# votnhan/VN_celeb_face_recognition

Measured on AMD Instinct MI355X. Metric: embeddings/sec @ bs=256 (InceptionResnetV1, 160x160), higher is better.
Workload: dtype bf16

## Files before the change

### vn_celeb_face_recognition_amd/csrc/conv_device.h

```cpp
#pragma once
#include <atomic>

#include "kernels.h"
#include "split_f16.h"

namespace vnf {

typedef __bf16 bf16x8_t __attribute__((ext_vector_type(8)));
typedef _Float16 f16x8_t __attribute__((ext_vector_type(8)));
typedef float f32x4_t __attribute__((ext_vector_type(4)));

struct KArgs {
  const char* x;
  const char* w;
  const float* bias;
  const int4* ktab;
  const char* res;
  const float* slope;
  const char* zero;
  int ldx, H, W, Ho, Wo, sh, sw, ph, pw;
  int K, Kpad, nkt;
  int wrs, wts;
  int ncls, cout_pad;
  int M, Cout, tiles_n, nblk;
// ... 324 lines not shown
  } else {
    for (int pass = 0; pass < EPASS; ++pass) {
      if ((wm * WTM) / RPP == pass) {
        const int rbase = wm * WTM - pass * RPP;
#pragma unroll
        for (int i = 0; i < TM; ++i)
#pragma unroll
          for (int j = 0; j < TN; ++j)
            *reinterpret_cast<f32x4_t*>(sC + (rbase + i * 16 + frow) * CST + wn * WTN + j * 16 + fgrp * 4) = acc[i][j];
      }
      __syncthreads();
#pragma unroll
      for (int it = 0; it < NIT; ++it) {
        const int idx = tid + it * NT;
        const int r = idx / CPR, cc = idx - r * CPR;
        const int m = m0 + pass * RPP + r, c = n0 + cc * 8;
        if (idx < RPP * CPR && m < a.M && c < a.Cout) {
          int sg = 0;
#pragma unroll
          for (int s = 1; s < 4; ++s)
            if (s < a.nseg && c >= a.seg_c0[s]) sg = s;
          float v[8];
          const f32x4_t v0 = *reinterpret_cast<const f32x4_t*>(sC + r * CST + cc * 8);
          const f32x4_t v1 = *reinterpret_cast<const f32x4_t*>(sC + r * CST + cc * 8 + 4);
          int cls = 0;
          if (a.ncls == 9) {
            const int rr = m % HoWo, ho = rr / a.Wo, wo = rr - ho * a.Wo;
            cls = (ho == 0 ? 0 : (ho == a.Ho - 1 ? 2 : 1)) * 3 + (wo == 0 ? 0 : (wo == a.Wo - 1 ? 2 : 1));
          }
          const float* bp = a.bias + (size_t)cls * a.cout_pad + c;
          const f32x4_t b0 = *reinterpret_cast<const f32x4_t*>(bp), b1 = *reinterpret_cast<const f32x4_t*>(bp + 4);
#pragma unroll
          for (int e = 0; e < 4; ++e) { v[e] = v0[e] + b0[e]; v[4 + e] = v1[e] + b1[e]; }
          if (a.res) {
            float rv[8];
            load8<T>(a.res + ((size_t)m * a.ldres + c) * ES, rv);
#pragma unroll
            for (int e = 0; e < 8; ++e) v[e] += rv[e];
          }
          if (a.act == ACT_RELU) {
#pragma unroll
            for (int e = 0; e < 8; ++e) v[e] = fmaxf(v[e], 0.f);
          } else if (a.act == ACT_PRELU) {
#pragma unroll
            for (int e = 0; e < 8; ++e) v[e] = v[e] > 0.f ? v[e] : v[e] * a.slope[c + e];
          }
          char* const dptr = a.seg_ptr[sg];
          if (a.out_f32)
            store8<float>(dptr + ((size_t)m * a.seg_ld[sg] + (c - a.seg_c0[sg])) * 4, v);
          else
            store8<T>(dptr + ((size_t)m * a.seg_ld[sg] + (c - a.seg_c0[sg])) * ES, v);
        }
      }
      __syncthreads();
    }
  }
}

__device__ __forceinline__ void glds16(const void* gsrc, unsigned lds_base) {
  unsigned keep;
  asm volatile(
      "s_mov_b32 %0, m0\n\ts_mov_b32 m0, %2\n\ts_nop 0\n\tglobal_load_lds_dwordx4 %1, off\n\ts_mov_b32 m0, %0"
      : "=&s"(keep)
      : "v"(gsrc), "s"(lds_base)
      : "memory");
}

template <int N>
__device__ __forceinline__ void wait_dma_and_barrier() {
  asm volatile("s_waitcnt vmcnt(%0) lgkmcnt(0)\n\ts_barrier" ::"n"(N) : "memory");
}

constexpr int patch_epi_bytes(int bm, int bn, int wm) {
  return bm * (bn + 4) * 4 <= 64 * 1024 ? bm * (bn + 4) * 4 : (bm / wm) * (bn + 4) * 4;
}
int patch_num_cfgs();
bool patch_cfg_ok(const ConvArgs& a, int pcfg);
hipError_t launch_patch(const ConvArgs& a, const KArgs& k, int pcfg, hipStream_t s);

int ws_num_cfgs();
bool ws_cfg_ok(const ConvArgs& a, int wcfg);
hipError_t launch_ws(const ConvArgs& a, const KArgs& k, int wcfg, hipStream_t s);

}
```

### vn_celeb_face_recognition_amd/csrc/conv_igemm.hip

```cpp
#include <mutex>
#include <type_traits>

#include "block35.h"
#include "conv_device.h"

namespace vnf {

template <int AP, int RS>
__device__ __forceinline__ void row_setup(const KArgs& a, int m0, int lrow, int (&abase)[AP], int (&ahi)[AP],
                                          int (&awi)[AP]) {
  const int HoWo = a.Ho * a.Wo;
#pragma unroll
  for (int p = 0; p < AP; ++p) {
    const int m = m0 + lrow + RS * p;
    if (m < a.M) {
      const int n = m / HoWo, r = m - n * HoWo;
      const int ho = r / a.Wo, wo = r - ho * a.Wo;
      ahi[p] = ho * a.sh - a.ph;
      awi[p] = wo * a.sw - a.pw;
      abase[p] = ((n * a.H + ahi[p]) * a.W + awi[p]) * a.ldx;
    } else {
      ahi[p] = -(1 << 24);
      awi[p] = 0;
      abase[p] = 0;
// ... 172 lines not shown
      rd(kt, 1, xf[1], wf[1]);
#pragma unroll
      for (int i = 0; i < TM; ++i)
#pragma unroll
        for (int j = 0; j < TN; ++j) mma_hh(acc[i][j], wh[c][j], xh[c][i]);
    };
    int kt = 0;
    for (; kt + 1 < nkt; kt += 2) {
      step(std::integral_constant<int, 0>{}, kt);
      step(std::integral_constant<int, 1>{}, kt + 1);
    }
    if (kt < nkt) {
      step(std::integral_constant<int, 0>{}, kt);
#pragma unroll
      for (int i = 0; i < TM; ++i)
#pragma unroll
        for (int j = 0; j < TN; ++j) mma_cross(acc[i][j], wh[0][j], wf[1][j], xh[0][i], xf[1][i]);
    } else {
#pragma unroll
      for (int i = 0; i < TM; ++i)
#pragma unroll
        for (int j = 0; j < TN; ++j) mma_cross(acc[i][j], wh[1][j], wf[1][j], xh[1][i], xf[1][i]);
    }
  } else {
    bool pend = false;
    for (int kt = 0; kt < nkt; ++kt) {
      sync_tile(kt);
      read_frags(kt, 0);
      if (pend) mma(1);
      pend = BKE / 2 < a.K - kt * BKE;
      if (pend) read_frags(kt, 1);
      mma(0);
    }
    if (pend) mma(1);
  }
  __syncthreads();
  conv_epilogue<T, BM, BN, WM, WN, S * STAGE>(a, acc, smem, m0, n0);
}

static const char* zero_page() {
  static char* z[16] = {nullptr};
  static std::once_flag once[16];
  int dev = 0;
  if (hipGetDevice(&dev) != hipSuccess || dev < 0 || dev >= 16) return nullptr;
  std::call_once(once[dev], [dev] {
    char* p = nullptr;
    if (hipMalloc((void**)&p, 256) != hipSuccess) return;
    (void)hipMemset(p, 0, 256);
    (void)hipDeviceSynchronize();
    z[dev] = p;
  });
  return z[dev];
}

const char* conv_zero_page() { return zero_page(); }

template <typename T, int BM, int BN, int WM, int WN, int S>
static hipError_t launch_dma(const KArgs& k, hipStream_t s) {
  allow_dynamic_lds<conv_igemm_dma_kernel<T, BM, BN, WM, WN, S>>(160 * 1024);
  KArgs kk = k;
  const int lds = S * (BM + BN) * 128;
  const int tiles_m = (k.M + BM - 1) / BM;
  kk.tiles_n = (k.Cout + BN - 1) / BN;
  kk.nblk = tiles_m * kk.tiles_n;
  hipLaunchKernelGGL((conv_igemm_dma_kernel<T, BM, BN, WM, WN, S>), dim3(kk.nblk), dim3(WM * WN * 64), lds, s, kk);
  return hipGetLastError();
}

struct TileCfg { int bm, bn, wm, wn, s; };
static const TileCfg kCfgs[] = {
    {128, 128, 2, 2, 3}, {128, 64, 2, 2, 3}, {128, 32, 4, 1, 3}, {64, 64, 2, 2, 4}, {64, 32, 2, 2, 4},
    {256, 32, 4, 1, 3},  {256, 64, 4, 1, 3}, {64, 128, 1, 4, 3}, {32, 64, 2, 2, 4}, {32, 128, 1, 4, 4},
    {128, 64, 2, 2, 4},  {64, 64, 2, 2, 3},  {128, 32, 4, 1, 4},
    {128, 128, 2, 4, 3}, {256, 128, 4, 2, 3}, {256, 64, 4, 2, 3}, {128, 64, 4, 2, 3}, {128, 256, 2, 4, 3},
    {128, 128, 2, 4, 4},
    {128, 64, 4, 2, 6},  {64, 64, 2, 2, 8},   {64, 32, 2, 2, 8},  {32, 64, 2, 2, 8},  {128, 32, 4, 1, 6},
    {64, 128, 2, 4, 5},  {128, 64, 2, 2, 6},
    {64, 256, 1, 8, 3},  {64, 256, 1, 8, 4},  {128, 256, 2, 4, 3},
    {128, 96, 4, 1, 3},  {64, 96, 2, 2, 4},   {128, 192, 2, 4, 3}, {64, 192, 2, 4, 3},  {256, 96, 4, 1, 3},
    {64, 192, 2, 4, 4},
};
constexpr int kNumCfgs = (int)(sizeof(kCfgs) / sizeof(kCfgs[0]));

int conv_num_cfgs() { return kNumCfgs + patch_num_cfgs() + ws_num_cfgs(); }

static bool dma_capable(const ConvArgs& a) { return (a.Kpad / (128 / dtype_size(a.dtype))) * 8 * 16 <= 24 * 1024; }

bool conv_cfg_ok(const ConvArgs& a, int cfg) {
  if (cfg >= kNumCfgs + patch_num_cfgs()) return dma_capable(a) && ws_cfg_ok(a, cfg - kNumCfgs - patch_num_cfgs());
  if (cfg >= kNumCfgs) return dma_capable(a) && patch_cfg_ok(a, cfg - kNumCfgs);
  if (cfg < 0) return false;
  const TileCfg& c = kCfgs[cfg];
  if (c.bn > 32 && a.Cout <= c.bn / 2) return false;
  if (((a.Cout + c.bn - 1) / c.bn) * c.bn > a.cout_pad) return false;
  if ((c.bn % 64) && a.Cout % c.bn) return false;
  const int lds = c.s * (c.bm + c.bn) * 128;
  return lds <= 160 * 1024;
}

template <typename T>
static hipError_t launch_cfg(int cfg, const KArgs& k, hipStream_t s) {
  switch (cfg) {
    case 0: return launch_dma<T, 128, 128, 2, 2, 3>(k, s);
    case 1: return launch_dma<T, 128, 64, 2, 2, 3>(k, s);
    case 2: return launch_dma<T, 128, 32, 4, 1, 3>(k, s);
    case 3: return launch_dma<T, 64, 64, 2, 2, 4>(k, s);
    case 4: return launch_dma<T, 64, 32, 2, 2, 4>(k, s);
    case 5: return launch_dma<T, 256, 32, 4, 1, 3>(k, s);
    case 6: return launch_dma<T, 256, 64, 4, 1, 3>(k, s);
    case 7: return launch_dma<T, 64, 128, 1, 4, 3>(k, s);
    case 8: return launch_dma<T, 32, 64, 2, 2, 4>(k, s);
    case 9: return launch_dma<T, 32, 128, 1, 4, 4>(k, s);
    case 10: return launch_dma<T, 128, 64, 2, 2, 4>(k, s);
    case 11: return launch_dma<T, 64, 64, 2, 2, 3>(k, s);
    case 12: return launch_dma<T, 128, 32, 4, 1, 4>(k, s);
    case 13: return launch_dma<T, 128, 128, 2, 4, 3>(k, s);
    case 14: return launch_dma<T, 256, 128, 4, 2, 3>(k, s);
    case 15: return launch_dma<T, 256, 64, 4, 2, 3>(k, s);
    case 16: return launch_dma<T, 128, 64, 4, 2, 3>(k, s);
    case 17: return launch_dma<T, 128, 256, 2, 4, 3>(k, s);
    case 18: return launch_dma<T, 128, 128, 2, 4, 4>(k, s);
    case 19: return launch_dma<T, 128, 64, 4, 2, 6>(k, s);
    case 20: return launch_dma<T, 64, 64, 2, 2, 8>(k, s);
    case 21: return launch_dma<T, 64, 32, 2, 2, 8>(k, s);
    case 22: return launch_dma<T, 32, 64, 2, 2, 8>(k, s);
    case 23: return launch_dma<T, 128, 32, 4, 1, 6>(k, s);
    case 24: return launch_dma<T, 64, 128, 2, 4, 5>(k, s);
    case 25: return launch_dma<T, 128, 64, 2, 2, 6>(k, s);
    case 26: return launch_dma<T, 64, 256, 1, 8, 3>(k, s);
    case 27: return launch_dma<T, 64, 256, 1, 8, 4>(k, s);
    case 28: return launch_dma<T, 128, 256, 2, 4, 3>(k, s);
    case 29: return launch_dma<T, 128, 96, 4, 1, 3>(k, s);
    case 30: return launch_dma<T, 64, 96, 2, 2, 4>(k, s);
    case 31: return launch_dma<T, 128, 192, 2, 4, 3>(k, s);
    case 32: return launch_dma<T, 64, 192, 2, 4, 3>(k, s);
    case 33: return launch_dma<T, 256, 96, 4, 1, 3>(k, s);
    case 34: return launch_dma<T, 64, 192, 2, 4, 4>(k, s);
  }
  return hipErrorInvalidValue;
}

template <typename T>
static hipError_t launch_typed(const ConvArgs& a, const KArgs& k, hipStream_t s) {
  if (!k.zero) return hipErrorOutOfMemory;
  if (a.cfg >= kNumCfgs + patch_num_cfgs() && conv_cfg_ok(a, a.cfg)) return launch_ws(a, k, a.cfg - kNumCfgs - patch_num_cfgs(), s);
  if (a.cfg >= kNumCfgs && conv_cfg_ok(a, a.cfg)) return launch_patch(a, k, a.cfg - kNumCfgs, s);
  if (a.cfg >= 0 && conv_cfg_ok(a, a.cfg)) return launch_cfg<T>(a.cfg, k, s);
  auto fits = [&](int) { return true; };
  int bn = 128;
  while (bn > 32 && !(fits(bn) && (a.Cout % bn == 0 || a.Cout > 2 * bn))) bn >>= 1;
  if (!fits(bn)) return hipErrorInvalidValue;
  auto blocks = [&](int bm_, int bn_) { return ((a.M + bm_ - 1) / bm_) * ((a.Cout + bn_ - 1) / bn_); };
  while (bn > 64 && blocks(128, bn) < 512) bn >>= 1;
  int bm = 128;
  if (bn <= 64 && blocks(128, bn) < 512) bm = 64;
  const int id = bm == 128 ? (bn == 128 ? 0 : bn == 64 ? 1 : 2) : (bn == 64 ? 3 : 4);
  return launch_cfg<T>(id, k, s);
}

hipError_t launch_conv(const ConvArgs& a, hipStream_t s) {
  if (a.M <= 0) return hipSuccess;
  const int es = dtype_size(a.dtype);
  const int bke = 128 / es;
  if (a.Cout % 8 || a.Kpad % bke || a.nseg < 1 || a.nseg > 4) return hipErrorInvalidValue;
  KArgs k;
  k.x = (const char*)a.x; k.w = (const char*)a.w; k.bias = a.bias; k.ktab = a.ktab;
  k.res = (const char*)a.res; k.slope = a.slope; k.zero = zero_page();
  k.ldx = a.ldx; k.H = a.H; k.W = a.W; k.Ho = a.Ho; k.Wo = a.Wo;
  k.sh = a.sh; k.sw = a.sw; k.ph = a.ph; k.pw = a.pw;
  k.K = a.K; k.Kpad = a.Kpad; k.nkt = a.Kpad / bke;
  k.wrs = a.Kpad * es; k.wts = 128;
  k.ncls = a.ncls; k.cout_pad = a.cout_pad;
  k.M = a.M; k.Cout = a.Cout; k.tiles_n = 0; k.nblk = 0;
  k.ldres = a.ldres; k.act = a.act; k.out_f32 = a.out_f32;
  k.nseg = a.nseg;
  k.KH = a.KH; k.KW = a.KW; k.Cin = a.Cin; k.pp = k.Wp = k.Hv = k.patch_bytes = k.lds_bytes = 0; k.dbg = nullptr;
  for (int i = 0; i < 4; ++i) {
    k.seg_c0[i] = i < a.nseg ? a.seg[i].c0 : 1 << 30;
    k.seg_c1[i] = i < a.nseg ? a.seg[i].c1 : 1 << 30;
    k.seg_ld[i] = i < a.nseg ? a.seg[i].ld : 0;
    k.seg_ptr[i] = i < a.nseg ? (char*)a.seg[i].ptr : nullptr;
  }
  switch (a.dtype) {
    case BF16: return launch_typed<__bf16>(a, k, s);
    case F16: return launch_typed<_Float16>(a, k, s);
    case F32: return launch_typed<float>(a, k, s);
    case F16X2: return launch_typed<sf16>(a, k, s);
    case F16P: return launch_typed<pf16>(a, k, s);
  }
  return hipErrorInvalidValue;
}

}
```

### vn_celeb_face_recognition_amd/csrc/engine.cpp

```cpp
#include "engine.h"
#include "split_f16.h"
#include "block35.h"
#include "stem_mid.h"
#include "trunk17.h"

#include <algorithm>
#include <cmath>
#include <cstdio>
#include <cstdlib>
#include <cstring>
#include <map>

namespace vnf {

static thread_local std::string g_err;
void set_error(const std::string& msg) { g_err = msg; }
int fail(int code, const std::string& msg) {
  g_err = msg;
  return code;
}
const char* last_error_cstr() { return g_err.c_str(); }

HandleBase::~HandleBase() {
  for (void* p : allocs) (void)hipFree(p);
// ... 25 lines not shown
    if (w[i].name) m[w[i].name] = &w[i];
}
const float* WeightMap::get(const std::string& name, int64_t numel) {
  auto it = m.find(name);
  if (it == m.end() || it->second->dtype != VNF_F32 || !it->second->data) {
    if (missing.empty()) missing = name;
    return nullptr;
  }
  int64_t n = 1;
  for (int i = 0; i < it->second->ndim; ++i) n *= it->second->shape[i];
  if (n != numel) {
    if (missing.empty()) missing = name + " (unexpected size)";
    return nullptr;
  }
  return (const float*)it->second->data;
}

static inline uint16_t f2bf16(float f) {
  uint32_t u;
  memcpy(&u, &f, 4);
  if ((u & 0x7fffffffu) > 0x7f800000u) return (uint16_t)((u >> 16) | 0x40);
  return (uint16_t)((u + 0x7fffu + ((u >> 16) & 1u)) >> 16);
}
void convert_to(int dtype, const float* src, void* dst, size_t n) {
  if (dtype == F32) {
    memcpy(dst, src, n * 4);
  } else if (dtype == BF16) {
    uint16_t* d = (uint16_t*)dst;
    for (size_t i = 0; i < n; ++i) d[i] = f2bf16(src[i]);
  } else if (dtype == F16X2) {
    sf16* d = (sf16*)dst;
    for (size_t i = 0; i < n; ++i) d[i] = sf16(src[i]);
  } else if (dtype == F16P) {
    _Float16* d = (_Float16*)dst;
    for (size_t t = 0; t + 32 <= n; t += 32)
      for (int i = 0; i < 32; ++i) {
        const sf16 v(src[t + i]);
        d[2 * t + i] = v.hi;
        d[2 * t + 32 + i] = v.lo;
      }
  } else {
    _Float16* d = (_Float16*)dst;
    for (size_t i = 0; i < n; ++i) d[i] = (_Float16)src[i];
  }
}

int Encoder::add_buf(int H, int W, int C) {
  Buf b;
  b.H = H; b.W = W; b.C = C;
  bufs.push_back(b);
  return (int)bufs.size() - 1;
}

ConvArgs Encoder::conv_args(const ConvLayer& L, int n0, int nn) const {
  const int es = dtype_size(dtype);
  const Buf& xb = bufs[L.x_buf];
  ConvArgs a;
  memset(&a, 0, sizeof(a));
  a.dtype = dtype;
  a.x = xb.ptr + ((size_t)n0 * xb.elems_per_image() + L.x_coff) * es;
  a.ldx = xb.C; a.H = L.H; a.W = L.W; a.Cin = L.cin; a.Ho = L.Ho; a.Wo = L.Wo;
  a.KH = L.KH; a.KW = L.KW; a.sh = L.sh; a.sw = L.sw; a.ph = L.ph; a.pw = L.pw;
  a.w = L.w; a.K = L.K; a.Kpad = L.Kpad; a.bias = L.bias; a.ncls = L.ncls; a.cout_pad = L.cout_pad;
  a.ktab = L.ktab; a.M = nn * L.Ho * L.Wo; a.Cout = L.cout; a.nseg = L.nseg;
  for (int i = 0; i < L.nseg; ++i) {
    a.seg[i].c0 = L.seg[i].c0; a.seg[i].c1 = L.seg[i].c1;
    if (L.seg[i].buf == -2) {
      a.seg[i].ptr = emb_raw + (size_t)n0 * 512;
      a.seg[i].ld = 512;
    } else {
      const Buf& ob = bufs[L.seg[i].buf];
      a.seg[i].ptr = ob.ptr + ((size_t)n0 * ob.elems_per_image() + L.seg[i].coff) * (L.out_f32 ? 4 : es);
      a.seg[i].ld = ob.C;
    }
  }
  if (L.res_buf >= 0) {
    const Buf& rb = bufs[L.res_buf];
    a.res = rb.ptr + ((size_t)n0 * rb.elems_per_image() + L.res_coff) * es;
    a.ldres = rb.C;
  }
  a.act = L.act; a.slope = L.slope; a.out_f32 = L.out_f32;
  a.cfg = L.cfg;
  a.ws_persist = env.ws_persist;
  return a;
}

int Encoder::autotune() {
  const int enabled = env.autotune, force = env.force_cfg;
  if (!enabled && force < -1) return VNF_OK;
  std::map<std::string, int> cache;
  const char* cache_path = env.tune_cache.empty() ? nullptr : env.tune_cache.c_str();
  bool cache_dirty = false;
  if (cache_path && enabled) {
    if (FILE* f = fopen(cache_path, "r")) {
      char key[256];
      int c;
      while (fscanf(f, "%255s %d", key, &c) == 2) cache[key] = c;
      fclose(f);
    }
  }
  VNF_HIP(hipDeviceSynchronize());
  struct Timers {
    hipEvent_t e0 = nullptr, e1 = nullptr;
    hipStream_t lane_s[4] = {nullptr, nullptr, nullptr, nullptr};
    hipEvent_t lane_e[4] = {nullptr, nullptr, nullptr, nullptr};
    ~Timers() {
      if (e0) (void)hipEventDestroy(e0);
      if (e1) (void)hipEventDestroy(e1);
      for (int l = 0; l < 4; ++l) {
        if (lane_e[l]) (void)hipEventDestroy(lane_e[l]);
        if (lane_s[l]) (void)hipStreamDestroy(lane_s[l]);
      }
    }
  } tm;
  VNF_HIP(hipEventCreate(&tm.e0));
  VNF_HIP(hipEventCreate(&tm.e1));
  hipEvent_t e0 = tm.e0, e1 = tm.e1;
  hipStream_t* lane_s = tm.lane_s;
  hipEvent_t* lane_e = tm.lane_e;
  const int lanes = env.tune_lanes > 0 ? (env.tune_lanes > 4 ? 4 : env.tune_lanes) : (tune_lanes < 1 ? 1 : tune_lanes);
  if (lanes > 1)
    for (int l = 0; l < lanes; ++l) {
      VNF_HIP(hipStreamCreateWithFlags(&lane_s[l], hipStreamNonBlocking));
      VNF_HIP(hipEventCreate(&lane_e[l]));
    }
  for (const Group& g : groups) {
    int part = (max_batch >= 192 && max_streams > 1) ? (max_batch + 1) / 2 : max_batch;
    if (tune_batch > 0 && tune_batch < part) part = tune_batch;
    const int nn = g.chunk < part ? g.chunk : part;
    for (int oi = g.first; oi < g.last; ++oi) {
      if (ops[oi].kind != Op::CONV) continue;
      bool in_fused = false;
      for (const FusedStack& f : fused) in_fused |= f.active && oi >= f.first && oi < (f.ext ? f.ext_last : f.last);
      if (in_fused) continue;
      ConvLayer& L = convs[ops[oi].a];
      float best = 1e30f;
      int best_cfg = -1;
      char key[256];
      snprintf(key, sizeof key, "%s/d%d/n%d/M%d/K%d/N%d/v%d/L%d", L.name.c_str(), dtype, nn, nn * L.Ho * L.Wo, L.Kpad, L.cout,
               conv_num_cfgs(), lanes);
      const auto hit = cache.find(key);
      if (hit != cache.end()) {
        ConvArgs a = conv_args(L, 0, nn);
        if (hit->second == -1 || conv_cfg_ok(a, hit->second)) { L.cfg = hit->second; continue; }
      }
      std::vector<std::pair<float, int>> timed;
      auto time_cfg = [&](const ConvArgs& a, int trials, int reps, float* out_ms) -> int {
        float ms = 1e30f;
        for (int trial = 0; trial < trials; ++trial) {
          float t = 0;
          if (lanes <= 1) {
            VNF_HIP(hipEventRecord(e0, 0));
            for (int r = 0; r < reps; ++r) (void)launch_conv(a, 0);
            VNF_HIP(hipEventRecord(e1, 0));
            VNF_HIP(hipEventSynchronize(e1));
            VNF_HIP(hipEventElapsedTime(&t, e0, e1));
          } else {
            VNF_HIP(hipDeviceSynchronize());
            VNF_HIP(hipEventRecord(e0, lane_s[0]));
            for (int r = 0; r < reps; ++r)
              for (int l = 0; l < lanes; ++l) (void)launch_conv(a, lane_s[l]);
            for (int l = 0; l < lanes; ++l) VNF_HIP(hipEventRecord(lane_e[l], lane_s[l]));
            for (int l = 0; l < lanes; ++l) {
              float tl = 0;
              VNF_HIP(hipEventSynchronize(lane_e[l]));
              VNF_HIP(hipEventElapsedTime(&tl, e0, lane_e[l]));
              if (tl > t) t = tl;
            }
          }
          t *= 4.f / reps;
          if (t < ms) ms = t;
        }
        *out_ms = ms;
        return VNF_OK;
      };
      const int logit = env.autotune_log;
      for (int cfg = -1; enabled && cfg < conv_num_cfgs(); ++cfg) {
        ConvArgs a = conv_args(L, 0, nn);
        a.cfg = cfg;
        if (cfg >= 0 && !conv_cfg_ok(a, cfg)) continue;
        if (launch_conv(a, 0) != hipSuccess) { (void)hipGetLastError(); continue; }
        float ms = 1e30f;
        const int rc = time_cfg(a, 2, 4, &ms);
        if (rc != VNF_OK) return rc;
        timed.emplace_back(ms, cfg);
        if (ms < best) { best = ms; best_cfg = cfg; }
        if (logit) fprintf(stderr, "autotune %s cfg %d: %.4f ms\n", L.name.c_str(), cfg, ms / 4);
      }
      if (env.tune_final && timed.size() > 1) {
        std::sort(timed.begin(), timed.end());
        float fbest = 1e30f;
        int fcfg = best_cfg, nfin = 0;
        for (const auto& tc : timed) {
          if (tc.first > timed[0].first * 1.08f || nfin == 4) break;
          ++nfin;
          ConvArgs a = conv_args(L, 0, nn);
          a.cfg = tc.second;
          float ms = 1e30f;
          const int rc = time_cfg(a, 3, 8, &ms);
          if (rc != VNF_OK) return rc;
          if (logit) fprintf(stderr, "autotune %s final cfg %d: %.4f ms\n", L.name.c_str(), tc.second, ms / 4);
          if (ms < fbest) { fbest = ms; fcfg = tc.second; }
        }
        if (nfin > 1) { best = fbest; best_cfg = fcfg; }
      }
      L.cfg = best_cfg;
      if (cache_path && enabled) { cache[key] = best_cfg; cache_dirty = true; }
      if (force >= -1) {
        ConvArgs a = conv_args(L, 0, nn);
        if (force == -1 || conv_cfg_ok(a, force)) L.cfg = force;
      }
    }
  }
  VNF_HIP(hipDeviceSynchronize());
  if (cache_dirty) {
    if (FILE* f = fopen(cache_path, "w")) {
      for (auto& kv : cache) fprintf(f, "%s %d\n", kv.first.c_str(), kv.second);
      fclose(f);
    }
  }
  return VNF_OK;
}

int Encoder::finalize() {
  const int es = dtype_size(dtype);
  for (auto& b : bufs) {
    const size_t bytes = b.elems_per_image() * es * (size_t)max_batch;
    b.ptr = (char*)dalloc(bytes);
    if (!b.ptr) return VNF_E_HIP;
    VNF_HIP(hipMemset(b.ptr, 0, bytes));
  }
  emb_raw = (float*)dalloc((size_t)max_batch * 512 * 4);
  if (!emb_raw) return VNF_E_HIP;
  macs_alg = macs_exec = 0;
  for (auto& c : convs) { macs_alg += c.macs_alg; macs_exec += c.macs_exec; }
  if (groups.empty()) groups.push_back({0, (int)ops.size(), 1 << 30});
  {
    const int rc = prepare_fused();
    if (rc != VNF_OK) return rc;
  }
  tune_dirty = true;
  return VNF_OK;
}

EncoderEnv EncoderEnv::read() {
  auto env_int = [](const char* name, int dflt) { const char* v = getenv(name); return v ? atoi(v) : dflt; };
  EncoderEnv e;
  e.fuse = env_int("VNF_FUSE", e.fuse);
  e.direct_stem = env_int("VNF_DIRECT_STEM", e.direct_stem);
  e.stem1a_mfma = env_int("VNF_STEM1A_MFMA", e.stem1a_mfma);
  e.stem_chunk = env_int("VNF_STEM_CHUNK", e.stem_chunk);
  e.ir100_chunk1 = env_int("VNF_IR100_CHUNK1", e.ir100_chunk1);
  e.ir100_chunk2 = env_int("VNF_IR100_CHUNK2", e.ir100_chunk2);
  e.retina_fuse = env_int("VNF_RETINA_FUSE", e.retina_fuse);
  e.ws_persist = env_int("VNF_WS_PERSIST", e.ws_persist);
  e.autotune = env_int("VNF_AUTOTUNE", e.autotune);
  e.force_cfg = env_int("VNF_FORCE_CFG", e.force_cfg);
  e.tune_lanes = env_int("VNF_TUNE_LANES", e.tune_lanes);
  e.autotune_log = env_int("VNF_AUTOTUNE_LOG", e.autotune_log);
  e.tune_final = env_int("VNF_TUNE_FINAL", 1) != 0;
  if (const char* cache = getenv("VNF_TUNE_CACHE")) e.tune_cache = cache;
  return e;
}

int Encoder::prepare_fused() {
  const int enabled = env.fuse;
  for (FusedStack& f : fused) {
    f.active = false;
    if (!enabled || (dtype != BF16 && dtype != F16 && dtype != F16P) || f.nblocks < 1 || f.nblocks > T17_MAX_BLOCKS) continue;
    if (f.kind == 2) {
      if (!(enabled & 4)) continue;
      const ConvLayer& c2a = convs[f.conv0];
      const ConvLayer& c2b = convs[f.conv0 + 1];
      if (c2a.cout != 32 || c2a.K != 288 || c2b.cout != 64 || c2b.K != 288 || c2a.ncls != 1 || c2b.ncls != 1)
        return fail(VNF_E_INVALID, "fused stem: unexpected layer shapes");
      StemMidPack pk;
      pk.w[0] = c2a.w; pk.kpad[0] = c2a.Kpad;
      pk.w[1] = c2b.w; pk.kpad[1] = c2b.Kpad;
      bool ext_ok = false;
      if ((enabled & 8) && f.ext_conv >= 0) {
        const ConvLayer& c3b = convs[f.ext_conv];
        ext_ok = c3b.cout == 80 && c3b.K == 64 && c3b.KH == 1 && c3b.ncls == 1 && c3b.nseg == 1 && c3b.res_buf < 0 && c3b.act == ACT_RELU &&
                 bufs[f.ext_out_buf].C == 80;
      }
      if (dtype == F16P && !ext_ok) continue;
      f.wstream = dalloc(dtype == F16P ? SMS_WFRAG_BYTES : SM_WFRAG_BYTES);
      f.bias = (float*)dalloc(SM_BIAS * 4);
      if (!f.wstream || !f.bias) return VNF_E_HIP;
      VNF_HIP(hipMemcpy(f.bias, c2a.bias, 32 * 4, hipMemcpyDeviceToDevice));
      VNF_HIP(hipMemcpy(f.bias + 32, c2b.bias, 64 * 4, hipMemcpyDeviceToDevice));
      VNF_HIP(dtype == F16P ? stem_mids_repack(pk, f.wstream, 0) : stem_mid_repack(pk, f.wstream, 0));
      VNF_HIP(hipDeviceSynchronize());
      f.macs_alg = c2a.macs_alg + c2b.macs_alg;
      f.active = true;
      f.ext = ext_ok;
      if (ext_ok) f.macs_alg += convs[f.ext_conv].macs_alg;
      continue;
    }
    if (f.kind == 35) {
      if (!(enabled & 2)) continue;
      std::vector<float> bias((size_t)f.nblocks * B35_BIAS, 0.f);
      static const int rows[5] = {96, 32, 32, 32, 256}, ks[5] = {256, 288, 288, 288, 96}, boff[5] = {0, 96, 128, 160, 192};
      const size_t wimg_bytes = dtype == F16P ? B35S_WIMG_BYTES : B35_WIMG_BYTES;
      f.wstream = dalloc((size_t)f.nblocks * wimg_bytes);
      f.bias = (float*)dalloc(bias.size() * 4);
      if (!f.wstream || !f.bias) return VNF_E_HIP;
      for (int b = 0; b < f.nblocks; ++b) {
        Block35Pack pk;
        pk.bias = f.bias + (size_t)b * B35_BIAS;
        for (int c = 0; c < 5; ++c) {
          const ConvLayer& L = convs[f.conv0 + 5 * b + c];
          if (L.cout != rows[c] || L.K != ks[c] || L.ncls != 1) return fail(VNF_E_INVALID, "fused Block35: unexpected layer shapes");
          pk.w[c] = L.w;
          pk.kpad[c] = L.Kpad;
          VNF_HIP(hipMemcpy(&bias[(size_t)b * B35_BIAS + boff[c]], L.bias, (size_t)rows[c] * 4, hipMemcpyDeviceToHost));
          f.macs_alg += L.macs_alg;
        }
        VNF_HIP(hipMemcpy(f.bias + (size_t)b * B35_BIAS, &bias[(size_t)b * B35_BIAS], (size_t)B35_BIAS * 4, hipMemcpyHostToDevice));
        VNF_HIP(dtype == F16P ? block35s_repack(pk, (char*)f.wstream + (size_t)b * wimg_bytes, 0)
                              : block35_repack(pk, (char*)f.wstream + (size_t)b * wimg_bytes, 0));
      }
      VNF_HIP(hipDeviceSynchronize());
      f.active = true;
      f.stack = (enabled & 16) && dtype != F16P;
      f.ext = false;
      if (f.stack && (enabled & 32) && f.ext_conv >= 0) {
        const ConvLayer& t = convs[f.ext_conv];
        const ConvLayer& last_up = convs[f.conv0 + 5 * (f.nblocks - 1) + 4];
        const bool ok = t.KH == 1 && t.KW == 1 && t.K == 256 && t.cout == 192 && t.ncls == 1 && t.nseg == 1 && t.res_buf < 0 &&
                        t.act == ACT_RELU && !t.out_f32 && t.x_buf == last_up.seg[0].buf && t.x_coff == 0 &&
                        t.seg[0].buf == f.ext_out_buf && t.seg[0].coff == 0 && bufs[f.ext_out_buf].C == 192;
        if (ok) {
          f.wtail = dalloc(B35_TAIL_BYTES);
          if (!f.wtail) return VNF_E_HIP;
          VNF_HIP(block35_tail_repack(t.w, t.Kpad, t.bias, f.wtail, 0));
          VNF_HIP(hipDeviceSynchronize());
          f.ext = true;
          f.macs_alg += t.macs_alg;
        }
      }
// ... 1139 lines not shown
```

### vn_celeb_face_recognition_amd/csrc/engine.h

```cpp
#pragma once
#include <hip/hip_runtime.h>
#include <stdint.h>

#include <string>
#include <unordered_map>
#include <vector>

#include "../../include/vnface.h"
#include "kernels.h"

namespace vnf {

void set_error(const std::string& msg);
int fail(int code, const std::string& msg);

#define VNF_HIP(expr)                                                                         \
  do {                                                                                        \
    hipError_t _e = (expr);                                                                   \
    if (_e != hipSuccess)                                                                     \
      return ::vnf::fail(VNF_E_HIP, std::string(#expr) + ": " + hipGetErrorString(_e));       \
  } while (0)

struct HandleBase {
  int kind = 0;
  int device = 0;
  std::vector<void*> allocs;
  virtual ~HandleBase();
  void* dalloc(size_t bytes);
  void* upload(const void* host, size_t bytes);
};

struct WeightMap {
  std::unordered_map<std::string, const vnf_tensor_desc*> m;
  std::string missing;
  WeightMap(const vnf_tensor_desc* w, int n);
  const float* get(const std::string& name, int64_t numel);
  bool has(const std::string& name) const { return m.count(name) != 0; }
};

void convert_to(int dtype, const float* src, void* dst, size_t n);

struct Buf {
  int H, W, C;
  size_t elems_per_image() const { return (size_t)H * W * C; }
  char* ptr = nullptr;
};

struct ConvLayer {
  std::string name;
  int x_buf, x_coff, cin;
  int H, W, Ho, Wo, KH, KW, sh, sw, ph, pw;
  void* w = nullptr;
  float* bias = nullptr;
  float* slope = nullptr;
  int4* ktab = nullptr;
  int K, Kpad, cout, cout_pad, ncls = 1;
  int nseg = 0;
  struct { int c0, c1, buf, coff; } seg[4];
  int res_buf = -1, res_coff = 0;
  int act = ACT_NONE, out_f32 = 0;
  int cfg = -1;
  double macs_alg = 0, macs_exec = 0;
};

struct Op {
  enum Kind { PACK, CONV, MAXPOOL, AVGPOOL, L2NORM, COPYOUT, MAXPOOLC, STEM1, DWCONV, UPADD, RSTEM, DWPW } kind;
  int a = 0, b = 0, c = 0, d = 0, e = 0;
};

struct DwLayer {
  int x_buf, o_buf, C, stride;
  float *w = nullptr, *bias = nullptr;
  float slope = 0.f;
};

struct DwPwLayer {
  int x_buf, o_buf, cin, cout, stride;
  float *dw = nullptr, *dbias = nullptr, *pw = nullptr, *pbias = nullptr;
  float slope = 0.f;
  std::string name;
};

struct Group { int first, last, chunk; };

struct FusedStack {
  int kind = 17;
  int first = 0, last = 0;
  int in_buf = -1, out_buf = -1;
  int nblocks = 0;
  int conv0 = 0;
  void* wstream = nullptr;
  float* bias = nullptr;
  void* wtail = nullptr;
  bool active = false;
  bool stack = false;
  double macs_alg = 0;
  int ext_last = 0, ext_conv = -1, ext_out_buf = -1;
  bool ext = false;
};

struct Tap { int buf, coff, C; };

struct EncoderEnv {
  int fuse = 31, direct_stem = 1, stem1a_mfma = 1, retina_fuse = 3, ws_persist = 1;
  int stem_chunk = 0, ir100_chunk1 = 0, ir100_chunk2 = 0;
  int autotune = 1, force_cfg = -2, tune_lanes = 0, autotune_log = 0;
  bool tune_final = true;
  std::string tune_cache;
  static EncoderEnv read();
};

struct Encoder : HandleBase {
  ~Encoder() override;
  int arch, dtype, max_batch, in_size;
  std::vector<Buf> bufs;
  std::vector<ConvLayer> convs;
  std::vector<DwLayer> dws;
  std::vector<DwPwLayer> dwpws;
  float *rstem_wa = nullptr, *rstem_bias = nullptr;
  std::vector<Op> ops;
  std::vector<Group> groups;
  std::vector<FusedStack> fused;
  int prepare_fused();
  std::unordered_map<std::string, Tap> taps;
  bool buf_materialised(int buf) const;
  float* emb_raw = nullptr;
  double macs_alg = 0, macs_exec = 0;

  int add_buf(int H, int W, int C);
  int finalize();
  int autotune();
  ConvArgs conv_args(const ConvLayer& L, int n0, int nn) const;
  int run(const void* x, int n, int x_dtype, float* out, hipStream_t s, std::string* report = nullptr);
  int run_range(const void* x, int i0, int i1, int x_dtype, float* out, hipStream_t s, std::string* report);
  float* stem_wt = nullptr;
  int n_ctx = 1, next_ctx = 0;
  std::vector<std::vector<char*>> ctx_bufs;
  std::vector<float*> ctx_emb;
  std::vector<hipEvent_t> ctx_ev;
  int select_ctx(hipStream_t s, int* used);
  int max_streams = 4;
  bool tune_dirty = true;
  int tune_lanes = 1;
  int tune_batch = 0;
  const EncoderEnv env = EncoderEnv::read();
  hipStream_t side[4] = {nullptr, nullptr, nullptr, nullptr};
  hipEvent_t join_ev[4] = {nullptr, nullptr, nullptr, nullptr}, fork_ev = nullptr;
};

int build_irv1(Encoder& e, WeightMap& wm);
int build_ir100(Encoder& e, WeightMap& wm);
int build_retina_mnet(Encoder& e, WeightMap& wm, int H, int W, int head_bufs[3]);
int build_rnet(Encoder& e, WeightMap& wm, bool mid);
int build_onet(Encoder& e, WeightMap& wm, bool mid);

}
```

### vn_celeb_face_recognition_amd/csrc/kernels.h

```cpp
#pragma once
#include <hip/hip_runtime.h>
#include <stdint.h>

namespace vnf {

enum DType { F32 = 0, BF16 = 1, F16 = 2, F16X2 = 5, F16P = 6 };
inline int dtype_size(int dt) { return (dt == F32 || dt == F16X2 || dt == F16P) ? 4 : 2; }
inline int dtype_chan_align(int dt) { return dt == F16P ? 8 : 16 / dtype_size(dt); }

enum Act { ACT_NONE = 0, ACT_RELU = 1, ACT_PRELU = 2 };

struct ConvSeg {
  int c0, c1;
  void* ptr;
  int ld;
};

struct ConvArgs {
  int dtype;
  const void* x;
  int ldx;
  int H, W, Cin;
  int Ho, Wo;
  int KH, KW, sh, sw, ph, pw;
  const void* w;
  int K, Kpad;
  const float* bias;
  int ncls;
  int cout_pad;
  const int4* ktab;
  int M, Cout;
  int nseg;
  ConvSeg seg[4];
  const void* res;
  int ldres;
  int act;
  const float* slope;
  int out_f32;
  int cfg;
  int ws_persist;
};

hipError_t launch_conv(const ConvArgs& a, hipStream_t s);
int conv_num_cfgs();
bool conv_cfg_ok(const ConvArgs& a, int cfg);

hipError_t launch_pack_input(const void* x, int x_dtype, void* out, int dtype, int n, int hw, hipStream_t s);

hipError_t launch_stem_conv1a(const void* x, int x_dtype, void* y, int ldy, int dtype, int n, const float* wt, bool mfma,
                              hipStream_t s);

hipError_t launch_maxpool3s2(const void* x, int ldx, void* y, int ldy, int dtype, int n, int H, int W, int C,
                             hipStream_t s);

hipError_t launch_maxpool_ceil(const void* x, int ldx, void* y, int ldy, int dtype, int n, int H, int W, int C, int k,
                               hipStream_t s);

hipError_t launch_avgpool(const void* x, int ldx, void* y, int dtype, int n, int HW, int C, hipStream_t s);

hipError_t launch_l2norm(const float* x, float* y, int n, int C, hipStream_t s);

hipError_t launch_logsoftmax_argmax(const float* logits, int ld, int C, int n, float* logp, int32_t* amax, float* prob,
                                    hipStream_t s);

hipError_t launch_dwconv3x3(const float* x, float* y, int n, int H, int W, int C, int stride, const float* w9c,
                            const float* bias, float slope, bool split, hipStream_t s);

hipError_t launch_retina_stem(const uint8_t* frames, int n, int H, int W, const float* wa, const float* bias, float slope, float* y,
                              bool split, hipStream_t s);
bool dwpw_supported(int cin, int cout);
hipError_t launch_dwpw(const float* x, float* y, int n, int H, int W, int cin, int cout, int stride, const float* dw, const float* dbias,
                       float dslope, const float* pw, const float* pbias, float pslope, bool split, hipStream_t s);

hipError_t launch_upsample_add(const float* x, int Hs, int Ws, float* y, int H, int W, int C, int n, bool split, hipStream_t s);

hipError_t launch_nhwc_to_nchw_f32(const void* x, int ldx, int dtype, float* y, int n, int HW, int C, hipStream_t s);

}
```

Baseline: 265,300.

## Add per-image windowed conv kernel with register-streamed weights as autotune option

Adds a new convolution kernel that assigns one workgroup per image, stages a padded row window of the input in LDS with double buffering, and streams prepacked weight fragments through a register ring while running MFMA. It targets 3x3 stride-1 ReLU convs whose Cout and Kpad match fixed shapes, aiming to reuse input across filter taps and avoid the im2col-style gather cost. Weights are repacked once at build time into a per-config layout. Autotune adds these configs and records a fallback tile config for batches too small for the image kernel. The cost is extra device memory, more autotune time and larger cache keys.

```diff
diff --git a/vn_celeb_face_recognition_amd/csrc/conv_device.h b/vn_celeb_face_recognition_amd/csrc/conv_device.h
--- a/vn_celeb_face_recognition_amd/csrc/conv_device.h
+++ b/vn_celeb_face_recognition_amd/csrc/conv_device.h
@@ -430,4 +430,8 @@
 bool ws_cfg_ok(const ConvArgs& a, int wcfg);
 hipError_t launch_ws(const ConvArgs& a, const KArgs& k, int wcfg, hipStream_t s);
 
-}
+int img_num_cfgs();
+bool img_cfg_ok(const ConvArgs& a, int icfg);
+hipError_t launch_img(const ConvArgs& a, const char* zero, int icfg, hipStream_t s);
+
+}
diff --git a/vn_celeb_face_recognition_amd/csrc/conv_igemm.hip b/vn_celeb_face_recognition_amd/csrc/conv_igemm.hip
--- a/vn_celeb_face_recognition_amd/csrc/conv_igemm.hip
+++ b/vn_celeb_face_recognition_amd/csrc/conv_igemm.hip
@@ -278,11 +278,13 @@
 };
 constexpr int kNumCfgs = (int)(sizeof(kCfgs) / sizeof(kCfgs[0]));
 
-int conv_num_cfgs() { return kNumCfgs + patch_num_cfgs() + ws_num_cfgs(); }
+int conv_first_img_cfg() { return kNumCfgs + patch_num_cfgs() + ws_num_cfgs(); }
+int conv_num_cfgs() { return conv_first_img_cfg() + img_num_cfgs(); }
 
 static bool dma_capable(const ConvArgs& a) { return (a.Kpad / (128 / dtype_size(a.dtype))) * 8 * 16 <= 24 * 1024; }
 
 bool conv_cfg_ok(const ConvArgs& a, int cfg) {
+  if (cfg >= conv_first_img_cfg()) return img_cfg_ok(a, cfg - conv_first_img_cfg());
   if (cfg >= kNumCfgs + patch_num_cfgs()) return dma_capable(a) && ws_cfg_ok(a, cfg - kNumCfgs - patch_num_cfgs());
   if (cfg >= kNumCfgs) return dma_capable(a) && patch_cfg_ok(a, cfg - kNumCfgs);
   if (cfg < 0) return false;
@@ -339,6 +341,12 @@
 template <typename T>
 static hipError_t launch_typed(const ConvArgs& a, const KArgs& k, hipStream_t s) {
   if (!k.zero) return hipErrorOutOfMemory;
+  if (a.cfg >= conv_first_img_cfg() && conv_cfg_ok(a, a.cfg)) {
+    if (a.M >= (long long)a.img_min * a.Ho * a.Wo) return launch_img(a, k.zero, a.cfg - conv_first_img_cfg(), s);
+    ConvArgs b = a;
+    b.cfg = a.cfg_alt < conv_first_img_cfg() ? a.cfg_alt : -1;
+    return launch_typed<T>(b, k, s);
+  }
   if (a.cfg >= kNumCfgs + patch_num_cfgs() && conv_cfg_ok(a, a.cfg)) return launch_ws(a, k, a.cfg - kNumCfgs - patch_num_cfgs(), s);
   if (a.cfg >= kNumCfgs && conv_cfg_ok(a, a.cfg)) return launch_patch(a, k, a.cfg - kNumCfgs, s);
   if (a.cfg >= 0 && conv_cfg_ok(a, a.cfg)) return launch_cfg<T>(a.cfg, k, s);
diff --git a/vn_celeb_face_recognition_amd/csrc/conv_img.hip b/vn_celeb_face_recognition_amd/csrc/conv_img.hip
--- /dev/null
+++ b/vn_celeb_face_recognition_amd/csrc/conv_img.hip
@@ -0,0 +1,297 @@
+#include <type_traits>
+
+#include "conv_device.h"
+
+namespace vnf {
+
+namespace {
+
+constexpr int IMG_RING = 8;
+constexpr int IMG_LDS_MAX = 160 * 1024;
+
+struct ImgArgs {
+  const char* x;
+  const uint4* wimg;
+  const float* bias;
+  const int4* ktab;
+  const char* zero;
+  char* y;
+  int ldx, ldy, H, W, Cin, Ho, Wo, ph, pw;
+  int pp, Wp;
+  int rpp, npass;
+  int win_slots;
+  int win_bytes;
+};
+
+struct ImgGeom { int pp, Wp, rpp, npass, tail_rows, win_slots, win_bytes, lds; };
+
+}
+
+template <typename T, int TCH, int PS, int NI, int NT, int NKS, bool PIPE>
+__global__ __launch_bounds__(512, 2) void conv_img_kernel(const ImgArgs a) {
+  extern __shared__ __attribute__((aligned(16))) char smem[];
+  constexpr int F = NKS * TCH;
+  static_assert(F % IMG_RING == 0 && F >= IMG_RING, "the ring slot of a fragment must not depend on the pass");
+  const int tid = threadIdx.x, lane = tid & 63;
+  const int wave = __builtin_amdgcn_readfirstlane(tid >> 6);
+  const int frow = lane & 15, fgrp = lane >> 4;
+  const int cg = wave / PS, part = wave % PS;
+  const int img = blockIdx.x;
+  const unsigned lds0 = (unsigned)reinterpret_cast<uintptr_t>((__attribute__((address_space(3))) char*)smem);
+
+  int* const sP = reinterpret_cast<int*>(smem + 2 * a.win_bytes);
+  const int zoff = 2 * a.win_bytes + NKS * 16;
+
+  const char* const ximg = a.x + (size_t)img * a.H * a.W * a.ldx * 2;
+  const int cpb = a.Cin / 8;
+  auto load_window = [&](int p) {
+    const int v0 = p * a.rpp;
+    const int npieces = a.win_bytes >> 10;
+    for (int pc = wave; pc < npieces; pc += 8) {
+      const int s = pc * 64 + lane;
+      const char* src = a.zero;
+      if (s < a.win_slots) {
+        const int px_ = s / a.pp, c = s - px_ * a.pp;
+        const int py = px_ / a.Wp, px = px_ - py * a.Wp;
+        const int iy = v0 + py - a.ph, ix = px - a.pw;
+        if (c < cpb && (unsigned)iy < (unsigned)a.H && (unsigned)ix < (unsigned)a.W)
+          src = ximg + (size_t)((iy * a.W + ix) * a.ldx) * 2 + c * 16;
+      }
+      glds16(src, __builtin_amdgcn_readfirstlane(lds0 + (unsigned)((p & 1) * a.win_bytes) + (unsigned)pc * 1024u));
+    }
+  };
+  load_window(0);
+
+  const char* const wgrp = reinterpret_cast<const char*>(a.wimg) + (size_t)cg * F * 1024;
+  const unsigned lane16_c = (unsigned)lane * 16u;
+  uint4 wq[IMG_RING];
+#pragma unroll
+  for (int r = 0; r < IMG_RING; ++r) wq[r] = *reinterpret_cast<const uint4*>(wgrp + (lane16_c + r * 1024u));
+
+  for (int i = tid; i < NKS * 4; i += 512) {
+    const int4 e = a.ktab[i];
+    const int cc = (e.x - (e.y * a.W + e.z) * a.ldx) / 8;
+    sP[i] = e.w ? ((e.y * a.Wp + e.z) * a.pp + cc) * 16 : -1;
+  }
+  if (tid < 4) reinterpret_cast<int*>(smem + zoff)[tid] = 0;
+
+  asm volatile("s_waitcnt vmcnt(0)" ::: "memory");
+  __syncthreads();
+
+  typedef T tx4 __attribute__((ext_vector_type(4)));
+  const int HoWo = a.Ho * a.Wo;
+
+  auto run_pass = [&](auto NIc, int p) {
+    constexpr int NIP = decltype(NIc)::value;
+    unsigned lane16 = lane16_c;
+    int q0 = part * 16 + frow;
+    asm volatile("" : "+v"(lane16), "+v"(q0));
+    const int rows = min(a.rpp, a.Ho - p * a.rpp);
+    const int npx = rows * a.Wo;
+    const int buf = (p & 1) * a.win_bytes;
+    int pb[NIP];
+#pragma unroll
+    for (int i = 0; i < NIP; ++i) {
+      const int q = min(q0 + 16 * PS * i, npx - 1);
+      const int oy = q / a.Wo, ox = q - oy * a.Wo;
+      pb[i] = buf + (oy * a.Wp + ox) * a.pp * 16;
+    }
+    f32x4_t acc[TCH][NIP];
+#pragma unroll
+    for (int j = 0; j < TCH; ++j)
+#pragma unroll
+      for (int i = 0; i < NIP; ++i) acc[j][i] = f32x4_t{0.f, 0.f, 0.f, 0.f};
+
+    auto read_frags = [&](uint4 (&xf)[NIP], int t) {
+#pragma unroll
+      for (int i = 0; i < NIP; ++i) xf[i] = *reinterpret_cast<const uint4*>(smem + (t >= 0 ? pb[i] + t : zoff));
+    };
+    auto mma_step = [&](int ks, const uint4 (&xf)[NIP]) {
+#pragma unroll
+      for (int j = 0; j < TCH; ++j) {
+        const int s = ks * TCH + j;
+#pragma unroll
+        for (int i = 0; i < NIP; ++i) mma_chunk<T>(acc[j][i], wq[s % IMG_RING], xf[i]);
+        wq[s % IMG_RING] = *reinterpret_cast<const uint4*>(wgrp + (lane16 + (unsigned)(((s + IMG_RING) % F) * 1024)));
+      }
+    };
+    int t = sP[fgrp];
+    if constexpr (PIPE) {
+      uint4 xf[2][NIP];
+      read_frags(xf[0], t);
+#pragma unroll
+      for (int ks = 0; ks < NKS; ++ks) {
+        if (ks + 1 < NKS) read_frags(xf[(ks + 1) & 1], sP[(ks + 1) * 4 + fgrp]);
+        mma_step(ks, xf[ks & 1]);
+        __builtin_amdgcn_sched_barrier(0);
+      }
+    } else {
+#pragma unroll
+      for (int ks = 0; ks < NKS; ++ks) {
+        const int tn = sP[((ks + 1) % NKS) * 4 + fgrp];
+        uint4 xf[NIP];
+        read_frags(xf, t);
+        mma_step(ks, xf);
+        t = tn;
+        __builtin_amdgcn_sched_barrier(0);
+      }
+    }
+
+    char* const yrow = a.y + ((size_t)img * HoWo + (size_t)p * a.rpp * a.Wo) * a.ldy * 2;
+    int qb = part * 16 + frow, eg = fgrp;
+    asm volatile("" : "+v"(qb), "+v"(eg));
+    f32x4_t bias[TCH];
+#pragma unroll
+    for (int j = 0; j < TCH; ++j) bias[j] = *reinterpret_cast<const f32x4_t*>(a.bias + (cg * TCH + j) * 16 + eg * 4);
+#pragma unroll
+    for (int j = 0; j + 1 < TCH; j += 2) {
+      const int c = (cg * TCH + j + (eg & 1)) * 16 + (eg >> 1) * 8;
+#pragma unroll
+      for (int i = 0; i < NIP; ++i) {
+        tx4 o0, o1;
+#pragma unroll
+        for (int e = 0; e < 4; ++e) {
+          o0[e] = (T)fmaxf(acc[j][i][e] + bias[j][e], 0.f);
+          o1[e] = (T)fmaxf(acc[j + 1][i][e] + bias[j + 1][e], 0.f);
+        }
+        const uint2 p0 = __builtin_bit_cast(uint2, o0), p1 = __builtin_bit_cast(uint2, o1);
+        const auto sx = __builtin_amdgcn_permlane16_swap(p0.x, p1.x, false, false);
+        const auto sy = __builtin_amdgcn_permlane16_swap(p0.y, p1.y, false, false);
+        const int q = qb + 16 * PS * i;
+        if (q < npx) *reinterpret_cast<uint4*>(yrow + (unsigned)(q * a.ldy + c) * 2u) = uint4{sx[0], sy[0], sx[1], sy[1]};
+      }
+    }
+    if constexpr (TCH % 2 == 1) {
+      constexpr int j = TCH - 1;
+      const int c = (cg * TCH + j) * 16 + eg * 4;
+#pragma unroll
+      for (int i = 0; i < NIP; ++i) {
+        tx4 o;
+#pragma unroll
+        for (int e = 0; e < 4; ++e) o[e] = (T)fmaxf(acc[j][i][e] + bias[j][e], 0.f);
+        const int q = qb + 16 * PS * i;
+        if (q < npx) *reinterpret_cast<uint2*>(yrow + (unsigned)(q * a.ldy + c) * 2u) = __builtin_bit_cast(uint2, o);
+      }
+    }
+  };
+
+  for (int p = 0; p < a.npass; ++p) {
+    if (p > 0) asm volatile("s_waitcnt lgkmcnt(0)\n\ts_barrier" ::: "memory");
+    if (p + 1 < a.npass) load_window(p + 1);
+    const int npx = min(a.rpp, a.Ho - p * a.rpp) * a.Wo;
+    if (npx <= PS * NT * 16)
+      run_pass(std::integral_constant<int, NT>{}, p);
+    else
+      run_pass(std::integral_constant<int, NI>{}, p);
+  }
+}
+
+__global__ void conv_img_repack_kernel(const char* __restrict__ w, int Kpad, int groups, int tch, int nks,
+                                       uint4* __restrict__ out) {
+  const int lane = threadIdx.x & 63;
+  const int frag = blockIdx.x * (blockDim.x >> 6) + (threadIdx.x >> 6);
+  const int F = nks * tch;
+  if (frag >= groups * F) return;
+  const int g = frag / F, s = frag - g * F;
+  const int ks = s / tch, j = s - ks * tch;
+  const int row = (g * tch + j) * 16 + (lane & 15), k = ks * 32 + 8 * (lane >> 4);
+  out[(size_t)frag * 64 + lane] = *reinterpret_cast<const uint4*>(w + ((size_t)row * Kpad + k) * 2);
+}
+
+struct ImgCfg { int tch, ps, ni, nt, nks; bool pipe; };
+static const ImgCfg kImg[] = {
+    {3, 2, 9, 5, 24, false},
+    {3, 2, 9, 5, 24, true},
+    {6, 4, 5, 3, 24, false},
+    {6, 4, 5, 3, 24, true},
+};
+constexpr int kNumImg = (int)(sizeof(kImg) / sizeof(kImg[0]));
+
+int img_num_cfgs() { return kNumImg; }
+
+static bool img_geom(const ConvArgs& a, const ImgCfg& c, ImgGeom& g) {
+  if (a.dtype != BF16 && a.dtype != F16) return false;
+  if (a.sh != 1 || a.sw != 1 || a.KH * a.KW <= 1 || a.Cin % 8) return false;
+  if (a.Ho != a.H + 2 * a.ph - a.KH + 1 || a.Wo != a.W + 2 * a.pw - a.KW + 1) return false;
+  if (a.nseg != 1 || a.seg[0].c0 != 0 || a.res || a.ncls != 1 || a.out_f32 || a.act != ACT_RELU) return false;
+  if (a.Cout % 64 || a.Cout != (8 / c.ps) * c.tch * 16 || a.Cout > a.cout_pad) return false;
+  if (a.Kpad != c.nks * 32) return false;
+  g.pp = a.Cin / 8;
+  while (g.pp % 4 != 2) ++g.pp;
+  g.Wp = a.W + 2 * a.pw;
+  g.rpp = (c.ps * c.ni * 16) / a.Wo;
+  if (g.rpp > a.Ho) g.rpp = a.Ho;
+  if (g.rpp < 1) return false;
+  if (g.rpp * a.Wo * 2 <= c.ps * c.ni * 16) return false;
+  g.npass = (a.Ho + g.rpp - 1) / g.rpp;
+  g.tail_rows = a.Ho - (g.npass - 1) * g.rpp;
+  g.win_slots = (g.rpp + a.KH - 1) * g.Wp * g.pp;
+  g.win_bytes = (g.win_slots + 63) / 64 * 1024;
+  g.lds = 2 * g.win_bytes + c.nks * 16 + 16;
+  return g.lds <= IMG_LDS_MAX;
+}
+
+static size_t img_stream_bytes(const ImgCfg& c) { return (size_t)(8 / c.ps) * c.tch * c.nks * 1024; }
+
+static long long img_stream_offset(const ConvArgs& a, int icfg) {
+  ImgGeom g;
+  if (icfg < 0 || icfg >= kNumImg || !img_geom(a, kImg[icfg], g)) return -1;
+  long long off = 0;
+  for (int i = 0; i < icfg; ++i)
+    if (img_geom(a, kImg[i], g)) off += (long long)img_stream_bytes(kImg[i]);
+  return off;
+}
+
+bool img_cfg_ok(const ConvArgs& a, int icfg) { return a.wimg && img_stream_offset(a, icfg) >= 0; }
+
+size_t conv_img_stream_bytes(const ConvArgs& a) {
+  size_t bytes = 0;
+  ImgGeom g;
+  for (int i = 0; i < kNumImg; ++i)
+    if (img_geom(a, kImg[i], g)) bytes += img_stream_bytes(kImg[i]);
+  return bytes;
+}
+
+hipError_t conv_img_repack(const ConvArgs& a, void* out, hipStream_t s) {
+  for (int i = 0; i < kNumImg; ++i) {
+    const long long off = img_stream_offset(a, i);
+    if (off < 0) continue;
+    const ImgCfg& c = kImg[i];
+    const int frags = (8 / c.ps) * c.nks * c.tch;
+    hipLaunchKernelGGL(conv_img_repack_kernel, dim3((frags + 3) / 4), dim3(256), 0, s, (const char*)a.w, a.Kpad, 8 / c.ps,
+                       c.tch, c.nks, (uint4*)((char*)out + off));
+    const hipError_t e = hipGetLastError();
+    if (e != hipSuccess) return e;
+  }
+  return hipSuccess;
+}
+
+template <typename T>
+static hipError_t launch_img_typed(int icfg, const ImgArgs& ia, int n, int lds, hipStream_t s) {
+  switch (icfg) {
+    case 0: return launch_with_lds<conv_img_kernel<T, 3, 2, 9, 5, 24, false>>(n, 512, lds, s, ia);
+    case 1: return launch_with_lds<conv_img_kernel<T, 3, 2, 9, 5, 24, true>>(n, 512, lds, s, ia);
+    case 2: return launch_with_lds<conv_img_kernel<T, 6, 4, 5, 3, 24, false>>(n, 512, lds, s, ia);
+    case 3: return launch_with_lds<conv_img_kernel<T, 6, 4, 5, 3, 24, true>>(n, 512, lds, s, ia);
+  }
+  return hipErrorInvalidValue;
+}
+
+hipError_t launch_img(const ConvArgs& a, const char* zero, int icfg, hipStream_t s) {
+  ImgGeom g;
+  const long long off = a.wimg ? img_stream_offset(a, icfg) : -1;
+  if (off < 0 || !zero || !img_geom(a, kImg[icfg], g)) return hipErrorInvalidValue;
+  const int n = a.M / (a.Ho * a.Wo);
+  if (n * a.Ho * a.Wo != a.M) return hipErrorInvalidValue;
+  ImgArgs ia;
+  ia.x = (const char*)a.x; ia.wimg = (const uint4*)((const char*)a.wimg + off); ia.bias = a.bias; ia.ktab = a.ktab;
+  ia.zero = zero; ia.y = (char*)a.seg[0].ptr;
+  ia.ldx = a.ldx; ia.ldy = a.seg[0].ld; ia.H = a.H; ia.W = a.W; ia.Cin = a.Cin; ia.Ho = a.Ho; ia.Wo = a.Wo;
+  ia.ph = a.ph; ia.pw = a.pw;
+  ia.pp = g.pp; ia.Wp = g.Wp; ia.rpp = g.rpp; ia.npass = g.npass; ia.win_slots = g.win_slots; ia.win_bytes = g.win_bytes;
+  if (a.dtype == BF16) return launch_img_typed<__bf16>(icfg, ia, n, g.lds, s);
+  if (a.dtype == F16) return launch_img_typed<_Float16>(icfg, ia, n, g.lds, s);
+  return hipErrorInvalidValue;
+}
+
+}
diff --git a/vn_celeb_face_recognition_amd/csrc/engine.cpp b/vn_celeb_face_recognition_amd/csrc/engine.cpp
--- a/vn_celeb_face_recognition_amd/csrc/engine.cpp
+++ b/vn_celeb_face_recognition_amd/csrc/engine.cpp
@@ -131,7 +131,26 @@
   a.act = L.act; a.slope = L.slope; a.out_f32 = L.out_f32;
   a.cfg = L.cfg;
   a.ws_persist = env.ws_persist;
+  a.wimg = L.wimg; a.img_min = img_min(); a.cfg_alt = L.cfg_alt;
   return a;
+}
+
+static const int kConvImgMinDefault = 64;
+int Encoder::img_min() const { return env.conv_img > 0 ? env.conv_img : kConvImgMinDefault; }
+
+int Encoder::prepare_conv_img() {
+  if (env.conv_img == 0) return VNF_OK;
+  for (ConvLayer& L : convs) {
+    const ConvArgs a = conv_args(L, 0, 1);
+    const size_t bytes = conv_img_stream_bytes(a);
+    if (!bytes) continue;
+    void* st = dalloc(bytes);
+    if (!st) return VNF_E_HIP;
+    VNF_HIP(conv_img_repack(a, st, 0));
+    L.wimg = st;
+  }
+  VNF_HIP(hipStreamSynchronize(0));
+  return VNF_OK;
 }
 
 int Encoder::autotune() {
@@ -188,11 +207,20 @@
       char key[256];
       snprintf(key, sizeof key, "%s/d%d/n%d/M%d/K%d/N%d/v%d/L%d", L.name.c_str(), dtype, nn, nn * L.Ho * L.Wo, L.Kpad, L.cout,
                conv_num_cfgs(), lanes);
+      const std::string alt_key = std::string(key) + "/alt";
       const auto hit = cache.find(key);
       if (hit != cache.end()) {
         ConvArgs a = conv_args(L, 0, nn);
-        if (hit->second == -1 || conv_cfg_ok(a, hit->second)) { L.cfg = hit->second; continue; }
-      }
+        const auto alt = cache.find(alt_key);
+        const bool is_img = hit->second >= conv_first_img_cfg();
+        if ((hit->second == -1 || conv_cfg_ok(a, hit->second)) && (!is_img || alt != cache.end())) {
+          L.cfg = hit->second;
+          L.cfg_alt = is_img ? alt->second : -1;
+          continue;
+        }
+      }
+      float best_tile = 1e30f;
+      int best_tile_cfg = -1;
       std::vector<std::pair<float, int>> timed;
       auto time_cfg = [&](const ConvArgs& a, int trials, int reps, float* out_ms) -> int {
         float ms = 1e30f;
@@ -228,12 +256,14 @@
         ConvArgs a = conv_args(L, 0, nn);
         a.cfg = cfg;
         if (cfg >= 0 && !conv_cfg_ok(a, cfg)) continue;
+        if (cfg >= conv_first_img_cfg() && nn < img_min()) continue;
         if (launch_conv(a, 0) != hipSuccess) { (void)hipGetLastError(); continue; }
         float ms = 1e30f;
         const int rc = time_cfg(a, 2, 4, &ms);
         if (rc != VNF_OK) return rc;
         timed.emplace_back(ms, cfg);
         if (ms < best) { best = ms; best_cfg = cfg; }
+        if (cfg < conv_first_img_cfg() && ms < best_tile) { best_tile = ms; best_tile_cfg = cfg; }
         if (logit) fprintf(stderr, "autotune %s cfg %d: %.4f ms\n", L.name.c_str(), cfg, ms / 4);
       }
       if (env.tune_final && timed.size() > 1) {
@@ -254,10 +284,18 @@
         if (nfin > 1) { best = fbest; best_cfg = fcfg; }
       }
       L.cfg = best_cfg;
-      if (cache_path && enabled) { cache[key] = best_cfg; cache_dirty = true; }
+      L.cfg_alt = best_cfg >= conv_first_img_cfg() ? best_tile_cfg : -1;
+      if (cache_path && enabled) {
+        cache[key] = best_cfg;
+        if (best_cfg >= conv_first_img_cfg()) cache[alt_key] = best_tile_cfg;
+        cache_dirty = true;
+      }
       if (force >= -1) {
         ConvArgs a = conv_args(L, 0, nn);
-        if (force == -1 || conv_cfg_ok(a, force)) L.cfg = force;
+        if (force == -1 || conv_cfg_ok(a, force)) {
+          L.cfg = force;
+          L.cfg_alt = force >= conv_first_img_cfg() ? best_tile_cfg : -1;
+        }
       }
     }
   }
@@ -285,7 +323,8 @@
   for (auto& c : convs) { macs_alg += c.macs_alg; macs_exec += c.macs_exec; }
   if (groups.empty()) groups.push_back({0, (int)ops.size(), 1 << 30});
   {
-    const int rc = prepare_fused();
+    int rc = prepare_fused();
+    if (rc == VNF_OK) rc = prepare_conv_img();
     if (rc != VNF_OK) return rc;
   }
   tune_dirty = true;
@@ -305,6 +344,7 @@
   e.ws_persist = env_int("VNF_WS_PERSIST", e.ws_persist);
   e.autotune = env_int("VNF_AUTOTUNE", e.autotune);
   e.force_cfg = env_int("VNF_FORCE_CFG", e.force_cfg);
+  e.conv_img = env_int("VNF_CONV_IMG", e.conv_img);
   e.tune_lanes = env_int("VNF_TUNE_LANES", e.tune_lanes);
   e.autotune_log = env_int("VNF_AUTOTUNE_LOG", e.autotune_log);
   e.tune_final = env_int("VNF_TUNE_FINAL", 1) != 0;
diff --git a/vn_celeb_face_recognition_amd/csrc/engine.h b/vn_celeb_face_recognition_amd/csrc/engine.h
--- a/vn_celeb_face_recognition_amd/csrc/engine.h
+++ b/vn_celeb_face_recognition_amd/csrc/engine.h
@@ -60,6 +60,8 @@
   int res_buf = -1, res_coff = 0;
   int act = ACT_NONE, out_f32 = 0;
   int cfg = -1;
+  int cfg_alt = -1;
+  void* wimg = nullptr;
   double macs_alg = 0, macs_exec = 0;
 };
 
@@ -105,6 +107,7 @@
   int fuse = 31, direct_stem = 1, stem1a_mfma = 1, retina_fuse = 3, ws_persist = 1;
   int stem_chunk = 0, ir100_chunk1 = 0, ir100_chunk2 = 0;
   int autotune = 1, force_cfg = -2, tune_lanes = 0, autotune_log = 0;
+  int conv_img = -1;
   bool tune_final = true;
   std::string tune_cache;
   static EncoderEnv read();
@@ -122,6 +125,8 @@
   std::vector<Group> groups;
   std::vector<FusedStack> fused;
   int prepare_fused();
+  int prepare_conv_img();
+  int img_min() const;
   std::unordered_map<std::string, Tap> taps;
   bool buf_materialised(int buf) const;
   float* emb_raw = nullptr;
diff --git a/vn_celeb_face_recognition_amd/csrc/kernels.h b/vn_celeb_face_recognition_amd/csrc/kernels.h
--- a/vn_celeb_face_recognition_amd/csrc/kernels.h
+++ b/vn_celeb_face_recognition_amd/csrc/kernels.h
@@ -39,11 +39,17 @@
   int out_f32;
   int cfg;
   int ws_persist;
+  const void* wimg;
+  int img_min;
+  int cfg_alt;
 };
 
 hipError_t launch_conv(const ConvArgs& a, hipStream_t s);
 int conv_num_cfgs();
+int conv_first_img_cfg();
 bool conv_cfg_ok(const ConvArgs& a, int cfg);
+size_t conv_img_stream_bytes(const ConvArgs& a);
+hipError_t conv_img_repack(const ConvArgs& a, void* out, hipStream_t s);
 
 hipError_t launch_pack_input(const void* x, int x_dtype, void* out, int dtype, int n, int hw, hipStream_t s);
 
```

Result: no change. 264,900 (-0.2%).
